# twmitchel/FieldConv

Measured on AMD Instinct MI355X. Metric: FieldConv fwd+bwd Medges/s (20k verts, k=32, C=48, M=2), higher is better.
Workload: dtype f32 (complex64 in/out; contractions on f16 MFMA with every operand split into two halves, fp32 accumulate)

## Files before the change

fieldconv_amd/_env.py:

```python
import os

SWITCHES = {
    'FC_MFMA': 'f32: fp32-MFMA contractions throughout; f16: single halves (reduced precision); default: split halves',
    'FC_RING': '0: frequency-major forward kernels for every mesh size; 2: ring-major ones for every size',
    'FC_GROUP_SPLIT': '0: the backward data kernel never runs the two frequency groups of a tile as separate work items; 2 (development): wherever legal',
    'FC_RING_COMPACT': '0: no compact LDS plans (aliased partials, half-size record chunks) for the ring-major forward kernel',
    'FC_RING_HALVES': '0: no half tiles in the last round of the ring-major forward kernel',
    'FC_HALF_TILES': '0: no half tiles in the frequency-major kernels; 2: half tiles in the backward kernels too',
    'FC_BWD_STREAM': '0: the data / filter kernel pair on large meshes too, instead of the H-streaming arrangement (gather + stream + gx kernels)',
    'FC_FILTER2': '0: the LDS-staged half-precision filter-gradient kernel instead of the register-fed one',
    'FC_SPLIT_FINISH': '1: partial sums and parameter-gradient chain as two launches',
    'FC_EDGE_PARTS_MAX': 'cap (log2) on the number of workgroups that share a tile on small meshes',
    'FC_ECHO_WPV': 'wavefronts per vertex in the ECHO descriptor kernels (1, 2 or 4)',
    'FC_STAMP_KERNEL': 'data | filter | stream: which backward kernel writes in-kernel time stamps (tools/stamps.py)',
    'FC_DEBUG': 'forward kernels: skip phases (WRONG RESULTS; refused by bench.py)',
    'FC_DEBUG_BWD': 'backward kernels: skip phases (bit 0 walk, bit 1 gxt product, bit 2 gW product, bit 3 H stores) (WRONG RESULTS; refused by bench.py)',
    'FC_LIN_DIRECT': '0: TangentLin on small meshes through the LDS-staged kernel instead of the direct one',
    'FC_DEBUG_RG': "ECHOBlock head's grouped GEMM: 1 no products, 2 no loads, 4 no staging (WRONG RESULTS; refused by bench.py)",
    'FC_DEBUG_RP': 'finishing launch: 1 no partial loads, 2 no parameter-gradient chain (WRONG RESULTS; refused by bench.py)',
    'FIELDCONV_DEV': '1: load libfieldconv_hip_dev.so (the library switches above exist there only; one of them set without this raises)',
    'FIELDCONV_HIP_LIB': 'path of a prebuilt libfieldconv_hip.so (development variants, fieldconv_amd.build.build_variant)',
    'FIELDCONV_DENSE': '1: FCPrecomp stencils through the dense-stencil kernels',
    'FIELDCONV_NO_GEO': '1: 64-byte factored records in the forward pass instead of geometric ones',
    'FIELDCONV_TORCH_GRAPH': '1: support graph built with torch ops instead of fc_graph_build',
    'FIELDCONV_NO_EDGE_SPLIT': '1: no edge split on small meshes',
    'FIELDCONV_EAGER_STENCIL': '1: FCPrecomp returns the dense (E,R,F) tensor',
    'FIELDCONV_NO_FUSED_EPILOGUE': '1: residual add and modReLU as separate operators',
    'FIELDCONV_SEPARATE_CALLS': '1: one foreign call per kernel instead of fc_forward_params / fc_backward_all',
    'FIELDCONV_CPP_NODES': '0: the block-level autograd nodes in Python (fieldconv_amd/blocks.py) instead of the C++ ones (fc_torch_nodes.so)',
    'FIELDCONV_ECHO_TAIL': "0: ECHOBlock's dense tail as torch's own Linear / ReLU autograd nodes instead of one node; aten: one node composed "
                           "of ATen GEMMs instead of the native head (fc_echo_head_*)",
    'FIELDCONV_BLOCK_CALLS': '0: FCResNetBlock / ECHOBlock / LiftBlock composed of per-operator autograd nodes instead of the block-level entry points',
    'BENCH_BACKEND': 'gloo: several ranks share a device (test rigs); default nccl (= RCCL)',
    'BENCH_FORCE_DIST': '1: run the partitioned / data-parallel code path with one rank',
    'BENCH_FORWARD_OVERLAP': '1: interior targets under the forward halo exchange',
    'BENCH_NO_OVERLAP': '1: gradient halo exchange not overlapped with the filter-gradient kernel',
    'BENCH_GRAPH_STEP': '1: the partitioned step captured in one HIP graph',
}

TEST_SWITCHES = {
    'FC_FULL_MODES': '1: tests/test_gpu_modes.py sweeps every development switch instead of the eight kernel-family / arithmetic modes',
    'FC_FUZZ_SHAPES': 'number of shapes in the seeded sweep against the oracle (default 40)',
    'FC_FUZZ_SEED': 'seed of that sweep',
    'FC_FUZZ_WIDE': '1: the sweep also draws layers wider than 64 channels and (n_rings, band_limit) pairs outside the compiled set',
    'FC_DIST_TEST_DEVICE': 'cuda: the distributed test worker runs the HIP kernels (two gloo ranks on one GPU)',
    'FC_DIST_OVERLAP': '0: the distributed test worker without forward / backward overlap',
    'FC_DIST_PLAN_ONLY': '1: the distributed test worker checks partition and halo plan at config-4 size only',
    'FC_DIST_CONFIG4': '1: the distributed GPU test worker runs config 4\'s per-rank size (20 000 owned vertices per rank)',
}

LIBRARY_SWITCHES = ('FC_BWD_STREAM', 'FC_RING', 'FC_GROUP_SPLIT', 'FC_RING_COMPACT', 'FC_RING_HALVES', 'FC_HALF_TILES', 'FC_FILTER2', 'FC_SPLIT_FINISH',
                    'FC_EDGE_PARTS_MAX', 'FC_ECHO_WPV', 'FC_STAMP_KERNEL', 'FC_DEBUG', 'FC_DEBUG_BWD', 'FC_DEBUG_RP', 'FC_DEBUG_RG', 'FC_LIN_DIRECT')

PREFIXES = ('FC_', 'FIELDCONV_', 'BENCH_')
WRONG_RESULTS = ('FC_DEBUG', 'FC_DEBUG_BWD', 'FC_DEBUG_RP', 'FC_DEBUG_RG')


def active(environ=None):
    environ = os.environ if environ is None else environ
    return {k: environ[k] for k in sorted(SWITCHES) if k in environ}


def unknown(environ=None):
    environ = os.environ if environ is None else environ
    return sorted(k for k in environ if k.startswith(PREFIXES) and k not in SWITCHES and k not in TEST_SWITCHES)
```

fieldconv_amd/csrc/fc_forward_ring.hip:

```cpp
#include <stdio.h>
#include "fc_forward_ring.hpp"
#include "fc_forward_kernels.hpp"

namespace fc {

bool ring_enabled(const fc_dims* d) {
    static const bool on = [] { const char* e = dev_env("FC_RING"); return !(e && atoi(e) == 0); }();
    return on && halves_of(d) == 2;
}

bool forward_ring_fits(const fc_dims* d) {
    static const bool force = [] { const char* e = dev_env("FC_RING"); return e && atoi(e) == 2; }();
    if (!ring_enabled(d) || !plan_ring(d->O, 2 * d->B + 1, d->I, halves_of(d)).ok) return false;
    return force || (d->N + kTile - 1) / kTile > num_cus();
}

void describe_forward(const fc_dims* d, int kind, char* buf, size_t n) {
    const char* mode = halves_of(d) == 2 ? "split-f16" : halves_of(d) == 1 ? "f16" : "f32";
    const char* rec = kind == 2 ? "geometric records" : kind == 1 ? "factored records" : "dense rows";
    if (kind != 0 && forward_ring_fits(d)) {
        const RingPlan p = plan_ring(d->O, 2 * d->B + 1, d->I, halves_of(d));
        snprintf(buf, n, "fc_forward_ring_kernel<%s,%s> (ring-major, 2 workgroups x 8 wavefronts per CU, %zu B LDS, %d %s record chunks%s)",
                 rec, mode, p.lds, p.nr, p.logh ? "half-size" : "1 KiB", p.alias ? ", partials aliased onto the slab" : "");
    } else {
        snprintf(buf, n, "%s<%s,%s> (frequency-major, 16 wavefronts per CU, parts=%d)", kind ? "fc_forward_factored_kernel" : "fc_forward_kernel",
                 rec, mode, 1 << forward_parts_log2(d, kind));
    }
}

size_t packed_ring_image_floats(int M, int F, int channels, int R, int halves) {
    const MmaGeom g = ring_geom(M, F, channels, halves);
    return (size_t)g.MP + (size_t)R * halves * g.MP * g.KP;
}

template <int R, int B, bool GEO, int LOGH>
static int launch_forward_ring(const float2* x, const float* rec, const fc_csr* g, const float* wpk, float2* y, const RingArgs& a,
                               size_t lds, int grid, hipStream_t stream) {
    auto kern = fc_forward_ring_kernel<R, B, GEO, LOGH>;
    static bool lds_ok[kMaxDevices] = {};
    if (!allow_full_lds(reinterpret_cast<const void*>(kern), lds, lds_ok)) return FC_ERR_LAUNCH;
    hipLaunchKernelGGL(kern, dim3(grid), dim3(kDuoThreads), lds, stream, x, rec, g->rowptr, g->runs, wpk, y, a);
    return hipGetLastError() == hipSuccess ? FC_OK : FC_ERR_LAUNCH;
}

int forward_ring_impl(const float* x, const float* rec, const fc_csr* g, const float* wpk, float* y, const fc_dims* d, int kind,
                      void* ws, size_t ws_bytes, const fc_epilogue* epi, hipStream_t stream) {
    const int F = 2 * d->B + 1;
    const RingPlan p = plan_ring(d->O, F, d->I, halves_of(d));
    if (!p.ok) return FC_ERR_UNSUPPORTED;
    RingArgs a;
    a.N = d->N; a.I = d->I; a.O = d->O;
    a.g = p.g;
    a.ntiles = (d->N + kTile - 1) / kTile;
    a.parts_log2 = (ws && ws_bytes >= forward_workspace_bytes_impl(d, kind)) ? forward_parts_log2(d, kind) : 0;
    a.part_stride = (uint32_t)forward_part_stride(d);
    a.epi = make_epi(epi);
    a.nr = p.nr;
    a.alias_part = p.alias;
    a.wpk_bytes = (uint32_t)(packed_ring_image_floats(d->O, F, d->I, d->R, p.g.split) * sizeof(float));
    a.slab_bytes_w = (uint32_t)(2 * p.g.split * p.g.MP * p.g.KP * 2);
    static const int dbg = [] { const char* e = dev_env("FC_DEBUG"); return e ? atoi(e) : 0; }();
    a.dbg = dbg;
    a.stamps = debug_stamp_buffer();
    const int nvt = a.ntiles << a.parts_log2;
    int grid = nvt < 2 * num_cus() ? nvt : 2 * num_cus();
    const int rem = nvt % grid;
    a.nv_full = nvt;
    a.nv_total = nvt;
    a.spread_cus = 0;
    static const bool halves = !(dev_env("FC_RING_HALVES") && atoi(dev_env("FC_RING_HALVES")) == 0);
    if (halves && a.parts_log2 == 0 && rem > 0 && 2 * rem <= grid) {
        a.nv_full = nvt - rem;
        a.nv_total = a.nv_full + 2 * rem;
    }
    const int cus = num_cus();
    if (halves && a.parts_log2 == 0 && nvt > cus && nvt < 2 * cus) {
        a.nv_full = 2 * nvt - 2 * cus;
        a.nv_total = 2 * cus;
        a.spread_cus = cus;
        grid = 2 * cus;
    }
    int rc = FC_ERR_UNSUPPORTED;
    const float2* x2 = reinterpret_cast<const float2*>(x);
    float2* y2 = reinterpret_cast<float2*>(a.parts_log2 ? static_cast<float*>(ws) : y);
#define FC_CASE(RR, BB)                                                                                            \
    if (d->R == RR && d->B == BB) {                                                                                \
        if constexpr (BB >= 2) {                                                                                   \
            if (p.logh)                                                                                            \
                rc = kind == 2 ? launch_forward_ring<RR, BB, true, 1>(x2, rec, g, wpk, y2, a, p.lds, grid, stream)  \
                               : launch_forward_ring<RR, BB, false, 1>(x2, rec, g, wpk, y2, a, p.lds, grid, stream); \
        }                                                                                                          \
        if (!p.logh)                                                                                               \
            rc = kind == 2 ? launch_forward_ring<RR, BB, true, 0>(x2, rec, g, wpk, y2, a, p.lds, grid, stream)      \
                           : launch_forward_ring<RR, BB, false, 0>(x2, rec, g, wpk, y2, a, p.lds, grid, stream);    \
    }
    FC_FOR_EACH_SHAPE(FC_CASE)
#undef FC_CASE
    if (rc != FC_OK || a.parts_log2 == 0) return rc;
    return sum_parts_epilogue(static_cast<const float*>(ws), y, (size_t)d->N * d->O, a.part_stride, 1 << a.parts_log2, d->O, a.epi, stream);
}

}
```

fieldconv_amd/csrc/fc_forward_ring.hpp:

```cpp
#pragma once
#include <stdlib.h>
#include "fc_common.hpp"
#include "fc_kernels.hpp"
#include "fc_tile.hpp"

namespace fc {

constexpr int kDuoWaves = 8;
constexpr int kDuoThreads = kDuoWaves * kWave;
constexpr size_t kDuoMaxLds = 80 * 1024;

struct RingArgs {
    int N, I, O;
    MmaGeom g;
    int ntiles;
    int parts_log2;
    uint32_t part_stride;
    int nr;
    int alias_part;
    int nv_full;
    int nv_total;
    int spread_cus;
    uint32_t wpk_bytes;
    uint32_t slab_bytes_w;
    int dbg;
    FwdEpi epi;
    unsigned long long* stamps;
};

__host__ __device__ inline MmaGeom ring_geom(int M, int F, int channels, int halves) {
    MmaGeom g = make_mma_geom(M, F, channels, halves);
    g.NKP = kDuoWaves / g.NMT;
    if (g.NKP > g.KST) g.NKP = g.KST;
    if (g.NKP < 1) g.NKP = 1;
    return g;
}

__device__ __forceinline__ int ring_item(const RingArgs& a) {
    if (a.spread_cus == 0) return first_tile_of_block();
    const int b = blockIdx.x, C = a.spread_cus, W = a.nv_full;
    if (b >= C) return a.nv_full + (C - W) + (b - C);
    const int w0 = (b * W) / C, w1 = ((b + 1) * W) / C;
    return w1 > w0 ? w0 : a.nv_full + (b - w0);
}

struct RingLds {
    float* slab;
    float* part;
    float* vinv;
    int* runs;
    float* ring;
};
__host__ __device__ inline size_t ring_lds_floats(const MmaGeom& g, int nr, int chunk_floats = 256, bool alias = false) {
    const size_t slab = slab_floats(g), part = partial_floats(g.NKP, g.MP);
    return (alias ? (slab > part ? slab : part) : slab + part) + kTile + kDuoWaves * 32 + (size_t)kDuoWaves * 2 * nr * chunk_floats;
}
__device__ __forceinline__ RingLds ring_lds(char* smem, const MmaGeom& g, bool alias) {
    RingLds l;
    l.slab = reinterpret_cast<float*>(smem);
    l.part = alias ? l.slab : l.slab + slab_floats(g);
    const size_t slab = slab_floats(g), part = partial_floats(g.NKP, g.MP);
    l.vinv = l.slab + (alias ? (slab > part ? slab : part) : slab + part);
    l.runs = reinterpret_cast<int*>(l.vinv + kTile);
    l.ring = reinterpret_cast<float*>(l.runs + kDuoWaves * 32);
    return l;
}

template <int R, int B, bool GEO, int LOGH = 0>
__global__ __launch_bounds__(kDuoThreads, 4) void fc_forward_ring_kernel(
    const float2* __restrict__ gx_, const float* __restrict__ grec, const int32_t* __restrict__ growptr,
    const int32_t* __restrict__ gruns, const float* __restrict__ gwpk, float2* __restrict__ gy_, const RingArgs a) {
    constexpr int F = 2 * B + 1;
    constexpr int RECF = GEO ? kGeoRecordFloats : factored_record_floats(B);
    constexpr int LOG_CR = (GEO ? kGeoLogChunkRecords : factored_log_chunk_records(B)) - LOGH;
    constexpr int CR = 1 << LOG_CR;
    constexpr int CHUNK = 256 >> LOGH;
    static_assert(LOG_CR >= 2, "a record chunk holds at least four records");
    extern __shared__ __attribute__((aligned(16))) char smem[];
    const MmaGeom& g = a.g;
    const RingLds l = ring_lds(smem, g, a.alias_part != 0);
    const int tid = threadIdx.x;
    const int lane = tid & 63;
    const int wave = __builtin_amdgcn_readfirstlane(tid >> 6);
    const int nr = a.nr;
    const int I = a.I;
    const int sfl = slab_floats(g);

    for (int idx = tid; idx < sfl; idx += kDuoThreads) l.slab[idx] = 0.f;
    __syncthreads();

    if (wave >= kDuoWaves / 2 && !(a.dbg & 4)) __builtin_amdgcn_s_setprio(1);
    Stamper stamp{(a.stamps && blockIdx.x == 0) ? a.stamps + wave * 256 : nullptr, 0};
    const int cl = lane < I ? lane : 0;
    const int mt = wave % g.NMT, kp = wave / g.NMT;
    const bool mma_active = kp < g.NKP;
    const rsrc_t wimg = make_rsrc(gwpk, a.wpk_bytes);
    const int planes0 = g.MP * 4;
    const int pl = a.parts_log2;
    const int nvt = a.ntiles << pl;

    auto ring_of = [&](const int j) { return l.ring + (wave * 2 + j) * nr * CHUNK; };
    auto dma_chunk = [&](const int j, const int first, const int ch) {
        const float* src = grec + ((size_t)first + (size_t)ch * CR) * RECF + lane * 4;
        if constexpr (LOGH == 0) lds_dma16_untracked(src, ring_of(j) + (ch & (nr - 1)) * CHUNK);
        else lds_dma16_untracked_lanes(src, ring_of(j) + (ch & (nr - 1)) * CHUNK, 0xffffffffull);
    };
    auto slot_range = [&](const int vt, const int j, const int par, int& b, int& e) {
        b = 0;
        e = 0;
        int run[R];
#pragma unroll
        for (int q = 0; q < R; ++q) run[q] = 0;
        int t = (vt >> pl) * kTile + wave + kDuoWaves * j;
        bool live = vt < nvt;
        if (vt >= a.nv_full) {
            const int h = vt - a.nv_full;
            t = (a.nv_full + (h >> 1)) * kTile + (h & 1) * kDuoWaves + wave;
            live = vt < a.nv_total && j == 0;
        }
        if (live && t < a.N) {
            const int rb = growptr[t];
            const int n = growptr[t + 1] - rb;
            const int part = vt & ((1 << pl) - 1);
            const int s0 = (n * part) >> pl, s1 = (n * (part + 1)) >> pl;
            b = rb + s0;
            e = rb + s1;
#pragma unroll
            for (int q = 0; q < R; ++q) run[q] = min(max(gruns[(size_t)t * kRunStride + q], s0), s1) - s0;
        }
        if (lane == 0) {
            int* lro = l.runs + (wave * 2 + j) * 16 + par * 8;
#pragma unroll
            for (int q = 0; q < R; ++q) lro[q] = run[q];
        }
    };
    auto rec_ptr = [&](const float* ring, const int s) {
        if constexpr (CR * RECF == CHUNK) return ring + ((s * RECF) & (nr * CHUNK - 1));
        else return ring + ((s >> LOG_CR) & (nr - 1)) * CHUNK + (s & (CR - 1)) * RECF;
    };
    auto first_rows = [&](const int j, const int nslots, float2& r0, float2& r1) {
        r0 = make_float2(0.f, 0.f);
        r1 = r0;
        if (nslots > 0) {
            const float* ring = ring_of(j);
            const int n0 = __float_as_int(ring[3]);
            const int n1 = __float_as_int(ring[min(1, nslots - 1) * RECF + 3]);
            r0 = gather_row(gx_, n0, 8u * I, 8u * cl);
            r1 = gather_row(gx_, n1, 8u * I, 8u * cl);
        }
    };

    int beg[2], end[2], par = 0;
#pragma unroll
    for (int j = 0; j < 2; ++j) {
        slot_range(ring_item(a), j, 0, beg[j], end[j]);
        const int nch = (end[j] - beg[j] + CR - 1) >> LOG_CR;
        for (int ch = 0; ch < min(nch, nr); ++ch) dma_chunk(j, beg[j], ch);
    }
    asm volatile("s_waitcnt vmcnt(0)" ::: "memory");
    float2 px[2][2];
#pragma unroll
    for (int j = 0; j < 2; ++j) first_rows(j, end[j] - beg[j], px[j][0], px[j][1]);

    f32x4 tot_re = {0.f, 0.f, 0.f, 0.f}, tot_im = tot_re;

    const int wv = ((mt * 16 + (lane & 15)) * 32 + 8 * (lane >> 4)) * 2;
    const int wplane = g.MP * g.KP * 2;
    const int wkb = g.MP * 64;
    u32x4 wf0[4], wf1[4];
    auto load_w = [&](const int rq, const int kb, u32x4 (&dst)[4]) {
        const int kc = min(kb, g.KST - 1);
        const int base = planes0 + rq * (int)a.slab_bytes_w + wkb * kc;
#pragma unroll
        for (int pnum = 0; pnum < 4; ++pnum) dst[pnum] = buffer_load16(wimg, wv, base + pnum * wplane);
    };
    auto prefetch_w = [&](const int rq) {
        if (mma_active) {
            load_w(rq, kp, wf0);
            load_w(rq, kp + g.NKP, wf1);
        } else {
            const u32x4 zero = {0u, 0u, 0u, 0u};
#pragma unroll
            for (int pnum = 0; pnum < 4; ++pnum) { wf0[pnum] = zero; wf1[pnum] = zero; }
        }
    };
    auto mma_block = [&](const lds_f16* sp, const int kb, const u32x4 (&w)[4], f32x4& are, f32x4& aim) {
        const int fr = lane & 15, fq = lane >> 4;
        const u32x4 sign = {0x80008000u, 0x80008000u, 0x80008000u, 0x80008000u};
        const lds_f16* s0 = sp + fr * g.KS + 32 * fq + 128 * kb;
        {
            const u32x4 srh = *reinterpret_cast<lds_u32x4*>(s0), srl = *reinterpret_cast<lds_u32x4*>(s0 + 8);
            are = mfma32h(w[1], srh, are); aim = mfma32h(w[3], srh, aim);
            are = mfma32h(w[0], srl, are); aim = mfma32h(w[2], srl, aim);
            are = mfma32h(w[0], srh, are); aim = mfma32h(w[2], srh, aim);
        }
        {
            u32x4 sih = *reinterpret_cast<lds_u32x4*>(s0 + 16), sil = *reinterpret_cast<lds_u32x4*>(s0 + 24);
            aim = mfma32h(w[1], sih, aim);
            aim = mfma32h(w[0], sil, aim);
            aim = mfma32h(w[0], sih, aim);
            sih ^= sign;
            sil ^= sign;
            are = mfma32h(w[3], sih, are);
            are = mfma32h(w[2], sil, are);
            are = mfma32h(w[2], sih, are);
        }
    };
    auto contract = [&](const int rq) {
        if (mma_active && !(a.dbg & 2)) {
            f32x4 tre = {0.f, 0.f, 0.f, 0.f}, tim = tre;
            const lds_f16* sp = (const lds_f16*)l.slab;
            for (int kb = kp; kb < g.KST; kb += 2 * g.NKP) {
                mma_block(sp, kb, wf0, tre, tim);
                if (kb + 2 * g.NKP < g.KST) load_w(rq, kb + 2 * g.NKP, wf0);
                if (kb + g.NKP < g.KST) {
                    mma_block(sp, kb + g.NKP, wf1, tre, tim);
                    if (kb + 3 * g.NKP < g.KST) load_w(rq, kb + 3 * g.NKP, wf1);
                }
            }
            const float inv = l.vinv[lane & 15];
            tot_re += tre * inv;
            tot_im += tim * inv;
        }
    };
    auto flush_row = [&](const f32x2 (&c)[F], const int j) {
        const int row_i = wave + kDuoWaves * j;
        float mx = 0.f;
#pragma unroll
        for (int f = 0; f < F; ++f) mx = fmaxf(mx, fmaxf(fabsf(c[f].x), fabsf(c[f].y)));
        mx = wave_max_nonneg(mx);
        float scale, inv;
        split_scale(mx, scale, inv);
        if (lane == 0) l.vinv[row_i] = inv;
        if (lane < g.KI) {
            lds_u32* const row = (lds_u32*)l.slab + row_i * (g.KS / 2);
            int o0 = split_pair_offset(lane, 2);
#pragma unroll
            for (int f = 0; f < F; ++f) {
                f16x2 hi, lo;
                split_halves2(c[f], scale, hi, lo);
                split_pair_store(row, o0, hi, lo, lane, 2);
                o0 += 2 * g.KI;
                asm volatile("" : "+v"(o0));
            }
        }
    };

    stamp.realtime(29);
    stamp(28);
    for (int vt = ring_item(a); vt < a.nv_total; vt += gridDim.x) {
        int nbeg[2], nend[2];
#pragma unroll
        for (int j = 0; j < 2; ++j) slot_range(vt + gridDim.x, j, par ^ 1, nbeg[j], nend[j]);

        f32x2 clo[2][F], chi[2][F];
#pragma unroll
        for (int j = 0; j < 2; ++j)
#pragma unroll
            for (int f = 0; f < F; ++f) { clo[j][f] = f32x2{0.f, 0.f}; chi[j][f] = clo[j][f]; }
        float2 xq[2][2] = {{px[0][0], px[0][1]}, {px[1][0], px[1][1]}};

        auto gather_run = [&](const int j, int s, const int run_end, f32x2 (&lo)[F], f32x2 (&hi)[F], float2& xe, float2& xo) {
            const float* const ring = ring_of(j);
            const int nslots = end[j] - beg[j];
            const int nch = (nslots + CR - 1) >> LOG_CR;
            auto slot = [&](const int s_, float2& xcur) {
                const float* rp = rec_ptr(ring, s_);
                const f32x4 head = *reinterpret_cast<const f32x4*>(rp);
                const int n2 = __float_as_int(rec_ptr(ring, min(s_ + 2, nslots - 1))[3]);
                const f32x2 w0v = f32x2{head.y, head.y}, w1v = f32x2{head.z, head.z};
                f32x2 z[F];
                if constexpr (GEO) {
                    const f32x4 cg = *reinterpret_cast<const f32x4*>(rp + 4);
                    rotate_geometric<B>(f32x2{xcur.x, xcur.y}, f32x2{cg.x, cg.y}, f32x2{cg.z, cg.w}, z);
                    xcur = gather_row(gx_, n2, 8u * I, 8u * cl);
                } else {
                    f32x2 xt[F], ph[F];
                    rotate_all<B>(f32x2{xcur.x, xcur.y}, xt);
                    xcur = gather_row(gx_, n2, 8u * I, 8u * cl);
#pragma unroll
                    for (int f = 0; f < F; ++f) {
                        ph[f] = *reinterpret_cast<const f32x2*>(rp + 4 + 2 * f);
                        z[f] = cmul_pk_step1(ph[f], xt[f]);
                    }
#pragma unroll
                    for (int f = 0; f < F; ++f) z[f] = cmul_pk_step2(ph[f], xt[f], z[f]);
                }
#pragma unroll
                for (int f = 0; f < F; ++f) lo[f] = __builtin_elementwise_fma(w0v, z[f], lo[f]);
#pragma unroll
                for (int f = 0; f < F; ++f) hi[f] = __builtin_elementwise_fma(w1v, z[f], hi[f]);
            };
            while (s < run_end) {
                const int m = s & (CR - 1);
                if (m == 0 && s > 0) {
                    const int ch = s >> LOG_CR;
                    asm volatile("s_waitcnt vmcnt(0)" ::: "memory");
                    if (ch - 1 + nr < nch) dma_chunk(j, beg[j], ch - 1 + nr);
                }
                int stop = min(run_end, s - m + CR);
                if (nr == 2) {
                    if (m == CR - 2) asm volatile("s_waitcnt vmcnt(0)" ::: "memory");
                    else if (m < CR - 2) stop = min(stop, s - m + CR - 2);
                }
                if ((s & 1) && s < stop) {
                    slot(s, xo);
                    ++s;
                }
                for (; s + 1 < stop; s += 2) {
                    slot(s, xe);
                    slot(s + 1, xo);
                }
                if (s < stop) {
                    slot(s, xe);
                    ++s;
                }
            }
        };

        stamp(10);
        for (int q = 0; q < R - 1; ++q) {
            if (!(a.dbg & 1)) {
#pragma unroll
                for (int j = 0; j < 2; ++j) {
                    const int* lro = l.runs + (wave * 2 + j) * 16 + par * 8;
                    const int s = __builtin_amdgcn_readfirstlane(lro[q]);
                    const int run_end = (q + 1 < R - 1) ? __builtin_amdgcn_readfirstlane(lro[q + 1]) : end[j] - beg[j];
                    gather_run(j, s, run_end, clo[j], chi[j], xq[j][0], xq[j][1]);
                }
            }
            stamp(0);
            if (q == R - 2) {
                asm volatile("s_waitcnt vmcnt(0)" ::: "memory");
#pragma unroll
                for (int j = 0; j < 2; ++j) {
                    const int nnch = (nend[j] - nbeg[j] + CR - 1) >> LOG_CR;
                    for (int ch = 0; ch < min(nnch, nr); ++ch) dma_chunk(j, nbeg[j], ch);
                }
            }
            prefetch_w(q);
            flush_row(clo[0], 0);
            if (vt < a.nv_full) flush_row(clo[1], 1);
            stamp(1);
            __syncthreads();
            stamp(2);
            contract(q);
            stamp(3);
            __syncthreads();
            stamp(4);
#pragma unroll
            for (int j = 0; j < 2; ++j)
#pragma unroll
                for (int f = 0; f < F; ++f) { clo[j][f] = chi[j][f]; chi[j][f] = f32x2{0.f, 0.f}; }
        }
        prefetch_w(R - 1);
        flush_row(clo[0], 0);
        if (vt < a.nv_full) flush_row(clo[1], 1);
        __syncthreads();
        asm volatile("s_waitcnt vmcnt(0)" ::: "memory");
#pragma unroll
        for (int j = 0; j < 2; ++j) {
            beg[j] = nbeg[j];
            end[j] = nend[j];
            first_rows(j, end[j] - beg[j], px[j][0], px[j][1]);
        }
        contract(R - 1);
        if (a.alias_part) __syncthreads();
        if (mma_active) store_partial(l.part, g, mt, kp, lane, tot_re, tot_im);
        tot_re = f32x4{0.f, 0.f, 0.f, 0.f};
        tot_im = tot_re;
        stamp(5);
        __syncthreads();
        {
            const bool half = vt >= a.nv_full;
            const int hh = vt - a.nv_full;
            const int row0 = half ? (a.nv_full + (hh >> 1)) * kTile + (hh & 1) * kDuoWaves : (vt >> pl) * kTile;
            const int nrows = half ? kDuoWaves : kTile;
            float2* const yout = gy_ + (size_t)(half ? 0 : (vt & ((1 << pl) - 1))) * a.part_stride;
            for (int idx = tid; idx < nrows * a.O; idx += kDuoThreads) {
                const int v = idx / a.O, o = idx - v * a.O;
                const int n = row0 + v;
                float2 sm = sum_partials(l.part, g, v, o);
                const float k = gwpk[o];
                sm.x *= k;
                sm.y *= k;
                if (n < a.N) {
                    if (pl == 0) sm = apply_epilogue(sm, (size_t)n * a.O + o, o, a.epi);
                    yout[(size_t)n * a.O + o] = sm;
                }
            }
        }
        if (a.alias_part) {
            __syncthreads();
            for (int idx = tid; idx < partial_floats(g.NKP, g.MP); idx += kDuoThreads) l.slab[idx] = 0.f;
            __syncthreads();
        }
        stamp(6);
        par ^= 1;
    }
    stamp(30);
    stamp.realtime(31);
}

struct RingPlan {
    MmaGeom g;
    int nr;
    int logh;
    int alias;
    size_t lds;
    bool ok;
};
inline RingPlan plan_ring(int M, int F, int channels, int halves) {
    RingPlan p;
    p.g = ring_geom(M, F, channels, halves);
    p.ok = false;
    p.nr = 0; p.lds = 0; p.logh = 0; p.alias = 0;
    if (halves != 2 || p.g.NMT > kDuoWaves) return p;
    static const bool compact = !(dev_env("FC_RING_COMPACT") && atoi(dev_env("FC_RING_COMPACT")) == 0);
    const int tries[4][3] = {{4, 0, 0}, {2, 0, 0}, {2, 0, 1}, {2, 1, 1}};
    for (int t = 0; t < (compact ? 4 : 2); ++t) {
        if (tries[t][1] && F < 5) continue;
        const size_t lds = ring_lds_floats(p.g, tries[t][0], 256 >> tries[t][1], tries[t][2] != 0) * sizeof(float);
        if (lds <= kDuoMaxLds) {
            p.nr = tries[t][0]; p.logh = tries[t][1]; p.alias = tries[t][2]; p.lds = lds; p.ok = true;
            break;
        }
    }
    return p;
}

}
```

Before: 1831.

## Add paired 16-wavefront ring-major forward kernel with 32-vertex items on large meshes

```diff
diff --git a/fieldconv_amd/_env.py b/fieldconv_amd/_env.py
--- a/fieldconv_amd/_env.py
+++ b/fieldconv_amd/_env.py
@@ -6,6 +6,7 @@
     'FC_GROUP_SPLIT': '0: the backward data kernel never runs the two frequency groups of a tile as separate work items; 2 (development): wherever legal',
     'FC_RING_COMPACT': '0: no compact LDS plans (aliased partials, half-size record chunks) for the ring-major forward kernel',
     'FC_RING_HALVES': '0: no half tiles in the last round of the ring-major forward kernel',
+    'FC_RING_PAIRS': '0: the 8-wavefront ring-major forward kernel on large meshes too, instead of the paired one (32-vertex items); 2: the paired one for any mesh size its plan fits',
     'FC_HALF_TILES': '0: no half tiles in the frequency-major kernels; 2: half tiles in the backward kernels too',
     'FC_BWD_STREAM': '0: the data / filter kernel pair on large meshes too, instead of the H-streaming arrangement (gather + stream + gx kernels)',
     'FC_FILTER2': '0: the LDS-staged half-precision filter-gradient kernel instead of the register-fed one',
@@ -49,7 +50,7 @@
     'FC_DIST_CONFIG4': '1: the distributed GPU test worker runs config 4\'s per-rank size (20 000 owned vertices per rank)',
 }
 
-LIBRARY_SWITCHES = ('FC_BWD_STREAM', 'FC_RING', 'FC_GROUP_SPLIT', 'FC_RING_COMPACT', 'FC_RING_HALVES', 'FC_HALF_TILES', 'FC_FILTER2', 'FC_SPLIT_FINISH',
+LIBRARY_SWITCHES = ('FC_BWD_STREAM', 'FC_RING', 'FC_GROUP_SPLIT', 'FC_RING_COMPACT', 'FC_RING_HALVES', 'FC_RING_PAIRS', 'FC_HALF_TILES', 'FC_FILTER2', 'FC_SPLIT_FINISH',
                     'FC_EDGE_PARTS_MAX', 'FC_ECHO_WPV', 'FC_STAMP_KERNEL', 'FC_DEBUG', 'FC_DEBUG_BWD', 'FC_DEBUG_RP', 'FC_DEBUG_RG', 'FC_LIN_DIRECT')
 
 PREFIXES = ('FC_', 'FIELDCONV_', 'BENCH_')
diff --git a/fieldconv_amd/csrc/fc_forward_ring.hip b/fieldconv_amd/csrc/fc_forward_ring.hip
--- a/fieldconv_amd/csrc/fc_forward_ring.hip
+++ b/fieldconv_amd/csrc/fc_forward_ring.hip
@@ -15,10 +15,20 @@
     return force || (d->N + kTile - 1) / kTile > num_cus();
 }
 
+bool forward_pairs_fits(const fc_dims* d) {
+    static const int mode = [] { const char* e = dev_env("FC_RING_PAIRS"); return e ? atoi(e) : 1; }();
+    if (mode == 0 || !forward_ring_fits(d) || !plan_ring_pairs(d->O, 2 * d->B + 1, d->I, halves_of(d)).ok) return false;
+    return mode == 2 || (d->N + 2 * kPairWaves - 1) / (2 * kPairWaves) > 2 * num_cus();
+}
+
 void describe_forward(const fc_dims* d, int kind, char* buf, size_t n) {
     const char* mode = halves_of(d) == 2 ? "split-f16" : halves_of(d) == 1 ? "f16" : "f32";
     const char* rec = kind == 2 ? "geometric records" : kind == 1 ? "factored records" : "dense rows";
-    if (kind != 0 && forward_ring_fits(d)) {
+    if (kind != 0 && forward_pairs_fits(d)) {
+        const RingPlan p = plan_ring_pairs(d->O, 2 * d->B + 1, d->I, halves_of(d));
+        snprintf(buf, n, "fc_forward_ring_kernel<%s,%s> (ring-major, paired: 1 workgroup x 16 wavefronts per CU, 32-vertex items, %zu B LDS, "
+                 "%d 1 KiB record chunks%s)", rec, mode, p.lds, p.nr, p.alias ? ", partials aliased onto the slab" : "");
+    } else if (kind != 0 && forward_ring_fits(d)) {
         const RingPlan p = plan_ring(d->O, 2 * d->B + 1, d->I, halves_of(d));
         snprintf(buf, n, "fc_forward_ring_kernel<%s,%s> (ring-major, 2 workgroups x 8 wavefronts per CU, %zu B LDS, %d %s record chunks%s)",
                  rec, mode, p.lds, p.nr, p.logh ? "half-size" : "1 KiB", p.alias ? ", partials aliased onto the slab" : "");
@@ -33,26 +43,28 @@
     return (size_t)g.MP + (size_t)R * halves * g.MP * g.KP;
 }
 
-template <int R, int B, bool GEO, int LOGH>
+template <int R, int B, bool GEO, int LOGH, int W = kDuoWaves>
 static int launch_forward_ring(const float2* x, const float* rec, const fc_csr* g, const float* wpk, float2* y, const RingArgs& a,
                                size_t lds, int grid, hipStream_t stream) {
-    auto kern = fc_forward_ring_kernel<R, B, GEO, LOGH>;
+    auto kern = fc_forward_ring_kernel<R, B, GEO, LOGH, W>;
     static bool lds_ok[kMaxDevices] = {};
     if (!allow_full_lds(reinterpret_cast<const void*>(kern), lds, lds_ok)) return FC_ERR_LAUNCH;
-    hipLaunchKernelGGL(kern, dim3(grid), dim3(kDuoThreads), lds, stream, x, rec, g->rowptr, g->runs, wpk, y, a);
+    hipLaunchKernelGGL(kern, dim3(grid), dim3(W * kWave), lds, stream, x, rec, g->rowptr, g->runs, wpk, y, a);
     return hipGetLastError() == hipSuccess ? FC_OK : FC_ERR_LAUNCH;
 }
 
 int forward_ring_impl(const float* x, const float* rec, const fc_csr* g, const float* wpk, float* y, const fc_dims* d, int kind,
                       void* ws, size_t ws_bytes, const fc_epilogue* epi, hipStream_t stream) {
     const int F = 2 * d->B + 1;
-    const RingPlan p = plan_ring(d->O, F, d->I, halves_of(d));
+    const bool pairs = forward_pairs_fits(d);
+    const RingPlan p = pairs ? plan_ring_pairs(d->O, F, d->I, halves_of(d)) : plan_ring(d->O, F, d->I, halves_of(d));
     if (!p.ok) return FC_ERR_UNSUPPORTED;
+    const int rows = pairs ? 2 * kPairWaves : kTile;
     RingArgs a;
     a.N = d->N; a.I = d->I; a.O = d->O;
     a.g = p.g;
-    a.ntiles = (d->N + kTile - 1) / kTile;
-    a.parts_log2 = (ws && ws_bytes >= forward_workspace_bytes_impl(d, kind)) ? forward_parts_log2(d, kind) : 0;
+    a.ntiles = (d->N + rows - 1) / rows;
+    a.parts_log2 = (!pairs && ws && ws_bytes >= forward_workspace_bytes_impl(d, kind)) ? forward_parts_log2(d, kind) : 0;
     a.part_stride = (uint32_t)forward_part_stride(d);
     a.epi = make_epi(epi);
     a.nr = p.nr;
@@ -63,7 +75,8 @@
     a.dbg = dbg;
     a.stamps = debug_stamp_buffer();
     const int nvt = a.ntiles << a.parts_log2;
-    int grid = nvt < 2 * num_cus() ? nvt : 2 * num_cus();
+    const int slots = pairs ? num_cus() : 2 * num_cus();
+    int grid = nvt < slots ? nvt : slots;
     const int rem = nvt % grid;
     a.nv_full = nvt;
     a.nv_total = nvt;
@@ -74,7 +87,7 @@
         a.nv_total = a.nv_full + 2 * rem;
     }
     const int cus = num_cus();
-    if (halves && a.parts_log2 == 0 && nvt > cus && nvt < 2 * cus) {
+    if (!pairs && halves && a.parts_log2 == 0 && nvt > cus && nvt < 2 * cus) {
         a.nv_full = 2 * nvt - 2 * cus;
         a.nv_total = 2 * cus;
         a.spread_cus = cus;
@@ -85,12 +98,17 @@
     float2* y2 = reinterpret_cast<float2*>(a.parts_log2 ? static_cast<float*>(ws) : y);
 #define FC_CASE(RR, BB)                                                                                            \
     if (d->R == RR && d->B == BB) {                                                                                \
+        if constexpr (2 * BB + 1 <= kPairMaxF) {                                                                   \
+            if (pairs)                                                                                             \
+                rc = kind == 2 ? launch_forward_ring<RR, BB, true, 0, kPairWaves>(x2, rec, g, wpk, y2, a, p.lds, grid, stream) \
+                               : launch_forward_ring<RR, BB, false, 0, kPairWaves>(x2, rec, g, wpk, y2, a, p.lds, grid, stream); \
+        }                                                                                                          \
         if constexpr (BB >= 2) {                                                                                   \
-            if (p.logh)                                                                                            \
+            if (!pairs && p.logh)                                                                                  \
                 rc = kind == 2 ? launch_forward_ring<RR, BB, true, 1>(x2, rec, g, wpk, y2, a, p.lds, grid, stream)  \
                                : launch_forward_ring<RR, BB, false, 1>(x2, rec, g, wpk, y2, a, p.lds, grid, stream); \
         }                                                                                                          \
-        if (!p.logh)                                                                                               \
+        if (!pairs && !p.logh)                                                                                     \
             rc = kind == 2 ? launch_forward_ring<RR, BB, true, 0>(x2, rec, g, wpk, y2, a, p.lds, grid, stream)      \
                            : launch_forward_ring<RR, BB, false, 0>(x2, rec, g, wpk, y2, a, p.lds, grid, stream);    \
     }
diff --git a/fieldconv_amd/csrc/fc_forward_ring.hpp b/fieldconv_amd/csrc/fc_forward_ring.hpp
--- a/fieldconv_amd/csrc/fc_forward_ring.hpp
+++ b/fieldconv_amd/csrc/fc_forward_ring.hpp
@@ -9,6 +9,8 @@
 constexpr int kDuoWaves = 8;
 constexpr int kDuoThreads = kDuoWaves * kWave;
 constexpr size_t kDuoMaxLds = 80 * 1024;
+constexpr int kPairWaves = 16;
+constexpr int kPairMaxF = 5;
 
 struct RingArgs {
     int N, I, O;
@@ -28,11 +30,15 @@
     unsigned long long* stamps;
 };
 
-__host__ __device__ inline MmaGeom ring_geom(int M, int F, int channels, int halves) {
+__host__ __device__ inline MmaGeom ring_geom(int M, int F, int channels, int halves, int waves = kDuoWaves) {
     MmaGeom g = make_mma_geom(M, F, channels, halves);
-    g.NKP = kDuoWaves / g.NMT;
+    g.NKP = waves / g.NMT;
     if (g.NKP > g.KST) g.NKP = g.KST;
     if (g.NKP < 1) g.NKP = 1;
+    if (waves != kDuoWaves) {
+        const int per = (g.KST + g.NKP - 1) / g.NKP;
+        g.NKP = (g.KST + per - 1) / per;
+    }
     return g;
 }
 
@@ -47,27 +53,31 @@
 struct RingLds {
     float* slab;
     float* part;
+    float* acc;
     float* vinv;
     int* runs;
     float* ring;
 };
-__host__ __device__ inline size_t ring_lds_floats(const MmaGeom& g, int nr, int chunk_floats = 256, bool alias = false) {
-    const size_t slab = slab_floats(g), part = partial_floats(g.NKP, g.MP);
-    return (alias ? (slab > part ? slab : part) : slab + part) + kTile + kDuoWaves * 32 + (size_t)kDuoWaves * 2 * nr * chunk_floats;
-}
+__host__ __device__ inline size_t ring_lds_floats(const MmaGeom& g, int nr, int chunk_floats = 256, bool alias = false, int waves = kDuoWaves) {
+    const size_t rt = waves / 8, slab = rt * slab_floats(g), part = partial_floats(g.NKP, g.MP);
+    return (alias ? (slab > part ? slab : part) : slab + part) + (rt - 1) * part + 2 * waves + waves * 32 + (size_t)waves * 2 * nr * chunk_floats;
+}
+template <int W = kDuoWaves>
 __device__ __forceinline__ RingLds ring_lds(char* smem, const MmaGeom& g, bool alias) {
+    constexpr int RT = W / 8;
     RingLds l;
     l.slab = reinterpret_cast<float*>(smem);
-    l.part = alias ? l.slab : l.slab + slab_floats(g);
-    const size_t slab = slab_floats(g), part = partial_floats(g.NKP, g.MP);
-    l.vinv = l.slab + (alias ? (slab > part ? slab : part) : slab + part);
-    l.runs = reinterpret_cast<int*>(l.vinv + kTile);
-    l.ring = reinterpret_cast<float*>(l.runs + kDuoWaves * 32);
+    const size_t slab = RT * slab_floats(g), part = partial_floats(g.NKP, g.MP);
+    l.part = alias ? l.slab : l.slab + slab;
+    l.acc = l.slab + (alias ? (slab > part ? slab : part) : slab + part);
+    l.vinv = l.acc + (RT - 1) * part;
+    l.runs = reinterpret_cast<int*>(l.vinv + 2 * W);
+    l.ring = reinterpret_cast<float*>(l.runs + W * 32);
     return l;
 }
 
-template <int R, int B, bool GEO, int LOGH = 0>
-__global__ __launch_bounds__(kDuoThreads, 4) void fc_forward_ring_kernel(
+template <int R, int B, bool GEO, int LOGH = 0, int W = kDuoWaves>
+__global__ __launch_bounds__(W * kWave, 4) void fc_forward_ring_kernel(
     const float2* __restrict__ gx_, const float* __restrict__ grec, const int32_t* __restrict__ growptr,
     const int32_t* __restrict__ gruns, const float* __restrict__ gwpk, float2* __restrict__ gy_, const RingArgs a) {
     constexpr int F = 2 * B + 1;
@@ -76,20 +86,26 @@
     constexpr int CR = 1 << LOG_CR;
     constexpr int CHUNK = 256 >> LOGH;
     static_assert(LOG_CR >= 2, "a record chunk holds at least four records");
+    static_assert(W == kDuoWaves || W == kPairWaves, "8 or 16 wavefronts");
+    constexpr int THREADS = W * kWave;
+    constexpr int ROWS = 2 * W;
+    constexpr int RT = ROWS / kTile;
+    constexpr bool LATE = W == kPairWaves;
     extern __shared__ __attribute__((aligned(16))) char smem[];
     const MmaGeom& g = a.g;
-    const RingLds l = ring_lds(smem, g, a.alias_part != 0);
+    const RingLds l = ring_lds<W>(smem, g, a.alias_part != 0);
     const int tid = threadIdx.x;
     const int lane = tid & 63;
     const int wave = __builtin_amdgcn_readfirstlane(tid >> 6);
     const int nr = a.nr;
     const int I = a.I;
-    const int sfl = slab_floats(g);
-
-    for (int idx = tid; idx < sfl; idx += kDuoThreads) l.slab[idx] = 0.f;
+    const int sfl = RT * slab_floats(g);
+    const int pfl = partial_floats(g.NKP, g.MP);
+
+    for (int idx = tid; idx < sfl; idx += THREADS) l.slab[idx] = 0.f;
     __syncthreads();
 
-    if (wave >= kDuoWaves / 2 && !(a.dbg & 4)) __builtin_amdgcn_s_setprio(1);
+    if (wave >= W / 2 && !(a.dbg & 4)) __builtin_amdgcn_s_setprio(1);
     Stamper stamp{(a.stamps && blockIdx.x == 0) ? a.stamps + wave * 256 : nullptr, 0};
     const int cl = lane < I ? lane : 0;
     const int mt = wave % g.NMT, kp = wave / g.NMT;
@@ -111,11 +127,11 @@
         int run[R];
 #pragma unroll
         for (int q = 0; q < R; ++q) run[q] = 0;
-        int t = (vt >> pl) * kTile + wave + kDuoWaves * j;
+        int t = (vt >> pl) * ROWS + wave + W * j;
         bool live = vt < nvt;
         if (vt >= a.nv_full) {
             const int h = vt - a.nv_full;
-            t = (a.nv_full + (h >> 1)) * kTile + (h & 1) * kDuoWaves + wave;
+            t = (a.nv_full + (h >> 1)) * ROWS + (h & 1) * W + wave;
             live = vt < a.nv_total && j == 0;
         }
         if (live && t < a.N) {
@@ -206,25 +222,56 @@
             are = mfma32h(w[2], sih, are);
         }
     };
-    auto contract = [&](const int rq) {
+    auto contract = [&](const int rq, const int nrt) {
         if (mma_active && !(a.dbg & 2)) {
-            f32x4 tre = {0.f, 0.f, 0.f, 0.f}, tim = tre;
             const lds_f16* sp = (const lds_f16*)l.slab;
-            for (int kb = kp; kb < g.KST; kb += 2 * g.NKP) {
-                mma_block(sp, kb, wf0, tre, tim);
-                if (kb + 2 * g.NKP < g.KST) load_w(rq, kb + 2 * g.NKP, wf0);
-                if (kb + g.NKP < g.KST) {
-                    mma_block(sp, kb + g.NKP, wf1, tre, tim);
-                    if (kb + 3 * g.NKP < g.KST) load_w(rq, kb + 3 * g.NKP, wf1);
-                }
-            }
-            const float inv = l.vinv[lane & 15];
-            tot_re += tre * inv;
-            tot_im += tim * inv;
+            if constexpr (RT == 1) {
+                f32x4 tre = {0.f, 0.f, 0.f, 0.f}, tim = tre;
+                for (int kb = kp; kb < g.KST; kb += 2 * g.NKP) {
+                    mma_block(sp, kb, wf0, tre, tim);
+                    if (kb + 2 * g.NKP < g.KST) load_w(rq, kb + 2 * g.NKP, wf0);
+                    if (kb + g.NKP < g.KST) {
+                        mma_block(sp, kb + g.NKP, wf1, tre, tim);
+                        if (kb + 3 * g.NKP < g.KST) load_w(rq, kb + 3 * g.NKP, wf1);
+                    }
+                }
+                const float inv = l.vinv[lane & 15];
+                tot_re += tre * inv;
+                tot_im += tim * inv;
+            } else {
+#pragma unroll
+                for (int rt = 0; rt < RT; ++rt) {
+                    if (rt < nrt) {
+                        f32x4 tre = {0.f, 0.f, 0.f, 0.f}, tim = tre;
+                        mma_block(sp + rt * kTile * g.KS, kp, wf0, tre, tim);
+                        if (kp + g.NKP < g.KST) mma_block(sp + rt * kTile * g.KS, kp + g.NKP, wf1, tre, tim);
+                        const float inv = l.vinv[rt * kTile + (lane & 15)];
+                        if (rt == 0) {
+                            tot_re += tre * inv;
+                            tot_im += tim * inv;
+                        } else {
+                            float* const pa = l.acc + (rt - 1) * pfl + (size_t)(kp * g.MP + mt * 16 + 4 * (lane >> 4)) * kPartStride + 2 * (lane & 15);
+                            f32x4 are = {0.f, 0.f, 0.f, 0.f}, aim = are;
+                            if (rq > 0) {
+#pragma unroll
+                                for (int j = 0; j < 4; ++j) {
+                                    const float2 v = *reinterpret_cast<const float2*>(pa + j * kPartStride);
+                                    are[j] = v.x;
+                                    aim[j] = v.y;
+                                }
+                            }
+                            are += tre * inv;
+                            aim += tim * inv;
+#pragma unroll
+                            for (int j = 0; j < 4; ++j) *reinterpret_cast<float2*>(pa + j * kPartStride) = make_float2(are[j], aim[j]);
+                        }
+                    }
+                }
+            }
         }
     };
     auto flush_row = [&](const f32x2 (&c)[F], const int j) {
-        const int row_i = wave + kDuoWaves * j;
+        const int row_i = wave + W * j;
         float mx = 0.f;
 #pragma unroll
         for (int f = 0; f < F; ++f) mx = fmaxf(mx, fmaxf(fabsf(c[f].x), fabsf(c[f].y)));
@@ -339,21 +386,28 @@
                 }
             }
             prefetch_w(q);
+            if (LATE) {
+                __syncthreads();
+                stamp(4);
+            }
             flush_row(clo[0], 0);
             if (vt < a.nv_full) flush_row(clo[1], 1);
             stamp(1);
             __syncthreads();
             stamp(2);
-            contract(q);
+            contract(q, vt < a.nv_full ? RT : 1);
             stamp(3);
-            __syncthreads();
-            stamp(4);
+            if (!LATE) {
+                __syncthreads();
+                stamp(4);
+            }
 #pragma unroll
             for (int j = 0; j < 2; ++j)
 #pragma unroll
                 for (int f = 0; f < F; ++f) { clo[j][f] = chi[j][f]; chi[j][f] = f32x2{0.f, 0.f}; }
         }
         prefetch_w(R - 1);
+        if (LATE) __syncthreads();
         flush_row(clo[0], 0);
         if (vt < a.nv_full) flush_row(clo[1], 1);
         __syncthreads();
@@ -364,7 +418,7 @@
             end[j] = nend[j];
             first_rows(j, end[j] - beg[j], px[j][0], px[j][1]);
         }
-        contract(R - 1);
+        contract(R - 1, vt < a.nv_full ? RT : 1);
         if (a.alias_part) __syncthreads();
         if (mma_active) store_partial(l.part, g, mt, kp, lane, tot_re, tot_im);
         tot_re = f32x4{0.f, 0.f, 0.f, 0.f};
@@ -374,13 +428,13 @@
         {
             const bool half = vt >= a.nv_full;
             const int hh = vt - a.nv_full;
-            const int row0 = half ? (a.nv_full + (hh >> 1)) * kTile + (hh & 1) * kDuoWaves : (vt >> pl) * kTile;
-            const int nrows = half ? kDuoWaves : kTile;
+            const int row0 = half ? (a.nv_full + (hh >> 1)) * ROWS + (hh & 1) * W : (vt >> pl) * ROWS;
+            const int nrows = half ? W : ROWS;
             float2* const yout = gy_ + (size_t)(half ? 0 : (vt & ((1 << pl) - 1))) * a.part_stride;
-            for (int idx = tid; idx < nrows * a.O; idx += kDuoThreads) {
+            for (int idx = tid; idx < nrows * a.O; idx += THREADS) {
                 const int v = idx / a.O, o = idx - v * a.O;
                 const int n = row0 + v;
-                float2 sm = sum_partials(l.part, g, v, o);
+                float2 sm = sum_partials(v < kTile ? l.part : l.acc + (v / kTile - 1) * pfl, g, v % kTile, o);
                 const float k = gwpk[o];
                 sm.x *= k;
                 sm.y *= k;
@@ -392,8 +446,8 @@
         }
         if (a.alias_part) {
             __syncthreads();
-            for (int idx = tid; idx < partial_floats(g.NKP, g.MP); idx += kDuoThreads) l.slab[idx] = 0.f;
-            __syncthreads();
+            for (int idx = tid; idx < pfl; idx += THREADS) l.slab[idx] = 0.f;
+            if (!LATE) __syncthreads();
         }
         stamp(6);
         par ^= 1;
@@ -428,5 +482,21 @@
     }
     return p;
 }
-
-}
+inline RingPlan plan_ring_pairs(int M, int F, int channels, int halves) {
+    RingPlan p;
+    p.g = ring_geom(M, F, channels, halves, kPairWaves);
+    p.ok = false;
+    p.nr = 0; p.lds = 0; p.logh = 0; p.alias = 0;
+    if (halves != 2 || F > kPairMaxF || p.g.NMT * p.g.NKP > kPairWaves || p.g.KST > 2 * p.g.NKP) return p;
+    const int tries[3][2] = {{4, 0}, {2, 0}, {2, 1}};
+    for (int t = 0; t < 3; ++t) {
+        const size_t lds = ring_lds_floats(p.g, tries[t][0], 256, tries[t][1] != 0, kPairWaves) * sizeof(float);
+        if (lds <= kMaxLds) {
+            p.nr = tries[t][0]; p.alias = tries[t][1]; p.lds = lds; p.ok = true;
+            break;
+        }
+    }
+    return p;
+}
+
+}
```

Result: faster. 1853, median of 6 (+1.2%).
